# joshuacwnewton/swiftwatcher

Measured on AMD Instinct MI355X. Metric: frames/sec (segment+classify) on 1080p ROI batches, higher is better.
Workload: dtype f64 (image_filtering), f32 (CNN)

## Files before the change

swiftwatcher_amd/csrc/cnn_poolsq.hip:

```cpp
#include "cnn_common.h"

namespace swk {

template <int PT, int NB>
__global__ __launch_bounds__(64 * PT * NB) void k_pool_squeeze(const float *__restrict__ src, int n, int T, int C, int P, const float *__restrict__ wgt,
                                                               const float *__restrict__ bias, int S, float *__restrict__ dst, int dH, int dW, int dC,
                                                               int off_y, int off_x, const float *__restrict__ ring, int live_lo, int live_n)
{
    constexpr int NW = PT * NB, NT = 64 * NW, PP = 32 * PT + 1, SP = 32 * NB + 1, KC = 32;
    __shared__ float sB[2][KC * PP];
    __shared__ float sA[2][KC * SP];
    const int tid = threadIdx.x, lane = tid & 63, wave = tid >> 6, r = lane & 31, hh = lane >> 5;
    const int pt = wave % PT, nb = wave / PT;
    const int npix = P * P, nchunk = C / KC;
    const int64_t rs = (int64_t)T * C;

    auto stage = [&](int seg, int c, int buf) {
        const int kb = c * KC;
        for (int i = tid; i < 32 * NB * 8; i += NT) {
            const int co = i >> 3, q = i & 7;
            float4 w = make_float4(0.f, 0.f, 0.f, 0.f);
            if (co < S) w = *(const float4 *)(wgt + (int64_t)co * C + kb + 4 * q);
            float *a = &sA[buf][(4 * q) * SP + co];
            a[0] = w.x; a[SP] = w.y; a[2 * SP] = w.z; a[3 * SP] = w.w;
        }
        const float *base = src + (int64_t)seg * T * rs + kb, *rbase = ring + kb;
        for (int i = tid; i < 32 * PT * 8; i += NT) {
            const int p = i >> 3, q = i & 7;
            float4 m = make_float4(0.f, 0.f, 0.f, 0.f);
            if (p < npix) {
                const int py = p / P, px = p - py * P;
                const int64_t o0 = (int64_t)(2 * py) * rs + (int64_t)(2 * px) * C + 4 * q;
                bool iny[3], inx[3];
#pragma unroll
                for (int d = 0; d < 3; ++d) {
                    iny[d] = (unsigned)(2 * py + d - live_lo) < (unsigned)live_n;
                    inx[d] = (unsigned)(2 * px + d - live_lo) < (unsigned)live_n;
                }
                m = *(const float4 *)((iny[0] && inx[0] ? base : rbase) + o0);
#pragma unroll
                for (int dy = 0; dy < 3; ++dy)
#pragma unroll
                    for (int dx = 0; dx < 3; ++dx) {
                        if (dy == 0 && dx == 0) continue;
                        const float4 v = *(const float4 *)((iny[dy] && inx[dx] ? base : rbase) + o0 + dy * rs + dx * C);
                        m.x = fmaxf(m.x, v.x); m.y = fmaxf(m.y, v.y); m.z = fmaxf(m.z, v.z); m.w = fmaxf(m.w, v.w);
                    }
            }
            float *b = &sB[buf][(4 * q) * PP + p];
            b[0] = m.x; b[PP] = m.y; b[2 * PP] = m.z; b[3 * PP] = m.w;
        }
    };

    for (int seg = blockIdx.x; seg < n; seg += gridDim.x) {
        f16v acc;
#pragma unroll
        for (int e = 0; e < 16; ++e) acc[e] = 0.0f;
        stage(seg, 0, 0);
        __syncthreads();
        for (int c = 0; c < nchunk; ++c) {
            const int buf = c & 1;
            if (c + 1 < nchunk) stage(seg, c + 1, buf ^ 1);
            const float *a = &sA[buf][(16 * hh) * SP + 32 * nb + r];
            const float *b = &sB[buf][(16 * hh) * PP + 32 * pt + r];
#pragma unroll
            for (int i = 0; i < 16; ++i) acc = __builtin_amdgcn_mfma_f32_32x32x2f32(a[i * SP], b[i * PP], acc, 0, 0, 0);
            __syncthreads();
        }
        const int p = 32 * pt + r;
        if (p < npix) {
            const int py = p / P, px = p - py * P;
            float *o = dst + (((int64_t)seg * dH + off_y + py) * dW + off_x + px) * dC + 32 * nb + 4 * hh;
#pragma unroll
            for (int g = 0; g < 4; ++g) {
                const int co = 32 * nb + 8 * g + 4 * hh;
                if (co < S) store_bias_relu(o + 8 * g, acc, g, *(const float4 *)(bias + co));
            }
        }
    }
}

template <int PT, int NB>
static int launch_pool_squeeze(hipStream_t s, const float *src, int n, int T, int C, int P, const float *wgt, const float *bias, int S, const Place &pl,
                               const float *ring, int live_lo, int live_n)
{
    int blocks = n < 256 * 8 ? n : 256 * 8;
    hipLaunchKernelGGL((k_pool_squeeze<PT, NB>), dim3((unsigned)blocks), dim3(64 * PT * NB), 0, s, src, n, T, C, P, wgt, bias, S, pl.dst, pl.dH, pl.dW,
                       pl.dC, pl.off_y, pl.off_x, ring, live_lo, live_n);
    return hipGetLastError() == hipSuccess ? SWK_OK : SWK_ERR_HIP;
}

}

#pragma GCC visibility push(default)
extern "C" {

int32_t swk_nhwc_maxpool3s2_conv1x1_bias_relu_place(void *stream, const float *src, int32_t n, int32_t t, int32_t cin, const float *weight,
                                                    const float *bias, int32_t cout, float *dst, int32_t dH, int32_t dW, int32_t dC,
                                                    int32_t off_y, int32_t off_x, const float *ring, int32_t live_lo, int32_t live_n)
{
    const int P = (t - 3) / 2 + 1;
    const swk::Place pl{dst, dH, dW, dC, off_y, off_x, 0};
    if (!src || !weight || !bias || n < 1 || t < 3 || cin < 32 || (cin & 31) || cout > 64 || P * P > 96 || !swk::place_ok(pl, P, P, cout, true) ||
        (((uintptr_t)src | (uintptr_t)weight | (uintptr_t)bias) & 15))
        return SWK_ERR_ARG;
    if (!ring) { ring = src; live_lo = 0; live_n = t; }
    if (live_lo < 0 || live_n < 0 || live_lo + live_n > t || ((uintptr_t)ring & 15)) return SWK_ERR_ARG;
    using namespace swk;
    hipStream_t s = (hipStream_t)stream;
    const int PT = (P * P + 31) / 32, NB = (cout + 31) / 32;
    if (PT == 1 && NB == 1) return launch_pool_squeeze<1, 1>(s, src, n, t, cin, P, weight, bias, cout, pl, ring, live_lo, live_n);
    if (PT == 2 && NB == 1) return launch_pool_squeeze<2, 1>(s, src, n, t, cin, P, weight, bias, cout, pl, ring, live_lo, live_n);
    if (PT == 3 && NB == 1) return launch_pool_squeeze<3, 1>(s, src, n, t, cin, P, weight, bias, cout, pl, ring, live_lo, live_n);
    if (PT == 1 && NB == 2) return launch_pool_squeeze<1, 2>(s, src, n, t, cin, P, weight, bias, cout, pl, ring, live_lo, live_n);
    if (PT == 2 && NB == 2) return launch_pool_squeeze<2, 2>(s, src, n, t, cin, P, weight, bias, cout, pl, ring, live_lo, live_n);
    if (PT == 3 && NB == 2) return launch_pool_squeeze<3, 2>(s, src, n, t, cin, P, weight, bias, cout, pl, ring, live_lo, live_n);
    return SWK_ERR_ARG;
}

}
#pragma GCC visibility pop
```

Baseline: 42590.

## Add persistent row-tiled maxpool+squeeze kernel with LDS-resident weights and pipelined loads

Adds a new fused maxpool3s2 + 1x1 conv kernel. It flattens all pooled pixels across segments into 32-row tiles, one tile per wave. Weights and bias are loaded once into dynamic LDS per persistent block. The 3x3 window loads are software-pipelined against the MFMA steps using sched_group_barriers, and magic-number division is used for pixel indexing. The aim is to stop restaging weights for every segment, fix poor wave utilisation when P*P is not a multiple of 32, and hide global load latency. The new path runs only for large batches that fit in LDS; otherwise the old per-segment kernel is used. It adds heavy register and LDS pressure and complexity.

```diff
diff --git a/swiftwatcher_amd/csrc/cnn_poolsq.hip b/swiftwatcher_amd/csrc/cnn_poolsq.hip
--- a/swiftwatcher_amd/csrc/cnn_poolsq.hip
+++ b/swiftwatcher_amd/csrc/cnn_poolsq.hip
@@ -2,10 +2,186 @@
 
 namespace swk {
 
+constexpr int POOLSQ_XP = 34;
+constexpr int POOLSQ_XFLOATS = 32 * POOLSQ_XP;
+
+template <int NBLK, int NWV>
+__global__ __launch_bounds__(64 * NWV, 3) void k_pool_squeeze(const float *__restrict__ src, int64_t rows, int T, int C, const float *__restrict__ wgt,
+                                                              const float *__restrict__ bias, int S, float *__restrict__ dst, int dH, int dW, int dC,
+                                                              int off_y, int off_x, const float *__restrict__ ring, int live_lo, int live_n,
+                                                              FastDiv fpp, FastDiv fp)
+{
+    constexpr int NP = 32 * NBLK, PITCH = NP + 1, NT = 64 * NWV, KC = 32, XP = POOLSQ_XP;
+    extern __shared__ float lds[];
+    const int tid = threadIdx.x, lane = tid & 63, r = lane & 31, hh = lane >> 5, q = lane & 7, pl = lane >> 3;
+    const int wave = __builtin_amdgcn_readfirstlane(tid >> 6);
+    float *lbias = lds + ((C * PITCH + 3) & ~3);
+    float *xw = lbias + NP + wave * POOLSQ_XFLOATS + (4 * q) * XP + pl;
+    const float *xr = lbias + NP + wave * POOLSQ_XFLOATS + (16 * hh) * XP + r;
+    const int P = (int)fp.d, nchunk = C / KC;
+    const int rs = T * C;
+    const int64_t ntiles = (rows + 31) >> 5, stride = (int64_t)gridDim.x * NWV;
+    int64_t tile = (int64_t)blockIdx.x * NWV + wave;
+
+    const float *lsrc[4];
+    int lwin[4];
+    unsigned lmask[4];
+    int lk = 0;
+    auto pixel = [&](unsigned t32, int j, unsigned &seg, unsigned &py, unsigned &px) -> bool {
+        asm volatile("" : "+s"(t32));
+        const unsigned m = t32 * 32u + (unsigned)j;
+        const bool valid = m < (unsigned)rows;
+        const unsigned mm = valid ? m : (unsigned)rows - 1u;
+        seg = fpp.div(mm);
+        const unsigned p = mm - seg * fpp.d;
+        py = fp.div(p);
+        px = p - py * (unsigned)P;
+        return valid;
+    };
+    auto locate = [&](int64_t t) {
+        int l = threadIdx.x & 63;
+        asm volatile("" : "+v"(l));
+#pragma unroll
+        for (int u = 0; u < 4; ++u) {
+            unsigned seg, py, px;
+            pixel((unsigned)t, 8 * u + (l >> 3), seg, py, px);
+            lwin[u] = (int)(2 * py) * rs + (int)(2 * px) * C + 4 * (l & 7);
+            lsrc[u] = src + (int64_t)seg * T * rs + lwin[u];
+            unsigned iny = 0, inx = 0;
+#pragma unroll
+            for (int d = 0; d < 3; ++d) {
+                iny |= (unsigned)((unsigned)(2 * py + d - live_lo) < (unsigned)live_n) << d;
+                inx |= (unsigned)((unsigned)(2 * px + d - live_lo) < (unsigned)live_n) << d;
+            }
+            lmask[u] = ((iny & 1u) ? inx : 0u) | ((iny & 2u) ? inx << 3 : 0u) | ((iny & 4u) ? inx << 6 : 0u);
+        }
+    };
+    float4 L[3][4];
+    float4 m[4];
+    auto issue = [&](int dy) {
+#pragma unroll
+        for (int u = 0; u < 4; ++u)
+#pragma unroll
+            for (int dx = 0; dx < 3; ++dx)
+                L[dx][u] = *(const float4 *)((((lmask[u] >> (3 * dy + dx)) & 1u) ? lsrc[u] : ring + lwin[u]) + (lk + dy * rs + dx * C));
+    };
+    auto max4 = [](const float4 a, const float4 b) { return make_float4(fmaxf(a.x, b.x), fmaxf(a.y, b.y), fmaxf(a.z, b.z), fmaxf(a.w, b.w)); };
+    auto fold = [&](bool first) {
+#pragma unroll
+        for (int u = 0; u < 4; ++u) m[u] = max4(max4(first ? L[0][u] : max4(m[u], L[0][u]), L[1][u]), L[2][u]);
+    };
+
+    locate(tile < ntiles ? tile : ntiles - 1);
+    issue(0);
+    for (int co = tid >> 4; co < NP; co += NT / 16)
+        for (int c4 = (tid & 15) * 4; c4 < C; c4 += 64) {
+            const float4 wv = co < S ? *(const float4 *)(wgt + (int64_t)co * C + c4) : make_float4(0.0f, 0.0f, 0.0f, 0.0f);
+            float *w = lds + c4 * PITCH + co;
+            w[0] = wv.x; w[PITCH] = wv.y; w[2 * PITCH] = wv.z; w[3 * PITCH] = wv.w;
+        }
+    for (int i = tid; i < NP; i += NT) lbias[i] = i < S ? bias[i] : 0.0f;
+    fold(true);
+    issue(1);
+    fold(false);
+    issue(2);
+    __syncthreads();
+
+    const float *wrow0 = lds + (16 * hh) * PITCH + r, *wrow = wrow0;
+    float bw[2][NBLK], bx[2];
+
+#define SWK_PS_STEPS(I0, I1)                                                                                                          \
+    _Pragma("unroll") for (int i = I0; i < I1; ++i) {                                                                                 \
+        if (i < 15) {                                                                                                                 \
+            _Pragma("unroll") for (int nb = 0; nb < NBLK; ++nb) bw[(i + 1) & 1][nb] = wrow[(i + 1) * PITCH + 32 * nb];                \
+            bx[(i + 1) & 1] = xr[(i + 1) * XP];                                                                                       \
+        }                                                                                                                             \
+        _Pragma("unroll") for (int nb = 0; nb < NBLK; ++nb) acc[nb] = __builtin_amdgcn_mfma_f32_32x32x2f32(bw[i & 1][nb], bx[i & 1], acc[nb], 0, 0, 0); \
+        if (i < 15) __builtin_amdgcn_sched_group_barrier(0x100 , NBLK + 1, 0);                                           \
+        __builtin_amdgcn_sched_group_barrier(0x008 , NBLK, 0);                                                              \
+    }
+
+    for (; tile < ntiles; tile += stride) {
+        const bool more = tile + stride < ntiles;
+        f16v acc[NBLK];
+#pragma unroll
+        for (int nb = 0; nb < NBLK; ++nb)
+#pragma unroll
+            for (int e = 0; e < 16; ++e) acc[nb][e] = 0.0f;
+        for (int c = 0; c < nchunk; ++c) {
+            fold(false);
+#pragma unroll
+            for (int u = 0; u < 4; ++u) {
+                xw[8 * u] = m[u].x; xw[XP + 8 * u] = m[u].y; xw[2 * XP + 8 * u] = m[u].z; xw[3 * XP + 8 * u] = m[u].w;
+            }
+            __builtin_amdgcn_wave_barrier();
+#pragma unroll
+            for (int nb = 0; nb < NBLK; ++nb) bw[0][nb] = wrow[32 * nb];
+            bx[0] = xr[0];
+            const bool last = c + 1 == nchunk;
+            if (!last) lk += KC;
+            else { lk = 0; locate(more ? tile + stride : tile); }
+            __builtin_amdgcn_sched_barrier(0);
+            issue(0);
+            __builtin_amdgcn_sched_barrier(0);
+            SWK_PS_STEPS(0, 5)
+            __builtin_amdgcn_sched_barrier(0);
+            fold(true);
+            issue(1);
+            __builtin_amdgcn_sched_barrier(0);
+            SWK_PS_STEPS(5, 10)
+            __builtin_amdgcn_sched_barrier(0);
+            fold(false);
+            issue(2);
+            __builtin_amdgcn_sched_barrier(0);
+            SWK_PS_STEPS(10, 16)
+            __builtin_amdgcn_sched_barrier(0);
+            wrow = last ? wrow0 : wrow + KC * PITCH;
+        }
+        unsigned seg, py, px;
+        int h4 = lane;
+        asm volatile("" : "+v"(h4));
+        const int rr = h4 & 31;
+        h4 = (h4 >> 5) * 4;
+        if (pixel((unsigned)tile, rr, seg, py, px)) {
+            float *o = dst + (((int64_t)seg * dH + off_y + py) * dW + off_x + px) * (int64_t)dC + h4;
+#pragma unroll
+            for (int nb = 0; nb < NBLK; ++nb)
+#pragma unroll
+                for (int g = 0; g < 4; ++g) {
+                    const int co = nb * 32 + 8 * g;
+                    if (co + h4 < S) store_bias_relu(o + co, acc[nb], g, *(const float4 *)(lbias + co + h4));
+                }
+        }
+    }
+#undef SWK_PS_STEPS
+}
+
+static size_t pool_squeeze_lds(int C, int nblk, int nwv)
+{
+    return (size_t)(((C * (32 * nblk + 1) + 3) & ~3) + 32 * nblk + nwv * POOLSQ_XFLOATS) * sizeof(float);
+}
+
+template <int NBLK, int NWV>
+static int launch_pool_squeeze_w(hipStream_t s, const float *src, int64_t rows, int T, int C, int P, const float *wgt, const float *bias, int S,
+                                 const Place &pl, const float *ring, int live_lo, int live_n)
+{
+    const size_t lds = pool_squeeze_lds(C, NBLK, NWV);
+    static unsigned long long attr_mask = 0;
+    if (!ensure_dyn_lds((const void *)k_pool_squeeze<NBLK, NWV>, 160 * 1024 - 256, attr_mask)) return SWK_ERR_HIP;
+    const int64_t ntiles = (rows + 31) / 32;
+    int64_t blocks = (ntiles + NWV - 1) / NWV;
+    const int64_t by_lds = (int64_t)((160 * 1024 - 256) / lds), by_waves = 12 / NWV;
+    const int64_t cap = 256 * (by_lds < by_waves ? by_lds : by_waves);
+    if (blocks > cap) blocks = cap;
+    hipLaunchKernelGGL((k_pool_squeeze<NBLK, NWV>), dim3((unsigned)blocks), dim3(64 * NWV), lds, s, src, rows, T, C, wgt, bias, S, pl.dst, pl.dH, pl.dW,
+                       pl.dC, pl.off_y, pl.off_x, ring, live_lo, live_n, FastDiv((unsigned)(P * P)), FastDiv((unsigned)P));
+    return hipGetLastError() == hipSuccess ? SWK_OK : SWK_ERR_HIP;
+}
+
 template <int PT, int NB>
-__global__ __launch_bounds__(64 * PT * NB) void k_pool_squeeze(const float *__restrict__ src, int n, int T, int C, int P, const float *__restrict__ wgt,
-                                                               const float *__restrict__ bias, int S, float *__restrict__ dst, int dH, int dW, int dC,
-                                                               int off_y, int off_x, const float *__restrict__ ring, int live_lo, int live_n)
+__global__ __launch_bounds__(64 * PT * NB) void k_pool_squeeze_seg(const float *__restrict__ src, int n, int T, int C, int P, const float *__restrict__ wgt,
+                                                                   const float *__restrict__ bias, int S, float *__restrict__ dst, int dH, int dW, int dC,
+                                                                   int off_y, int off_x, const float *__restrict__ ring, int live_lo, int live_n)
 {
     constexpr int NW = PT * NB, NT = 64 * NW, PP = 32 * PT + 1, SP = 32 * NB + 1, KC = 32;
     __shared__ float sB[2][KC * PP];
@@ -81,13 +257,32 @@
 }
 
 template <int PT, int NB>
-static int launch_pool_squeeze(hipStream_t s, const float *src, int n, int T, int C, int P, const float *wgt, const float *bias, int S, const Place &pl,
-                               const float *ring, int live_lo, int live_n)
+static int launch_pool_squeeze_seg(hipStream_t s, const float *src, int n, int T, int C, int P, const float *wgt, const float *bias, int S, const Place &pl,
+                                   const float *ring, int live_lo, int live_n)
 {
     int blocks = n < 256 * 8 ? n : 256 * 8;
-    hipLaunchKernelGGL((k_pool_squeeze<PT, NB>), dim3((unsigned)blocks), dim3(64 * PT * NB), 0, s, src, n, T, C, P, wgt, bias, S, pl.dst, pl.dH, pl.dW,
+    hipLaunchKernelGGL((k_pool_squeeze_seg<PT, NB>), dim3((unsigned)blocks), dim3(64 * PT * NB), 0, s, src, n, T, C, P, wgt, bias, S, pl.dst, pl.dH, pl.dW,
                        pl.dC, pl.off_y, pl.off_x, ring, live_lo, live_n);
     return hipGetLastError() == hipSuccess ? SWK_OK : SWK_ERR_HIP;
+}
+
+
+static bool pool_squeeze_by_row_tiles(int n, int P, int C, int nblk, int &nwv)
+{
+    const int64_t rows = (int64_t)n * P * P, ntiles = (rows + 31) / 32;
+    nwv = 12;
+    while (nwv > 3 && pool_squeeze_lds(C, nblk, nwv) > 160 * 1024 - 256) nwv /= 2;
+    return pool_squeeze_lds(C, nblk, nwv) <= 160 * 1024 - 256 && rows <= (int64_t)0x7fffff00 && ntiles >= 2 * 256 * nwv;
+}
+
+template <int NBLK>
+static int launch_pool_squeeze(hipStream_t s, const float *src, int n, int T, int C, int P, int nwv, const float *wgt, const float *bias, int S,
+                               const Place &pl, const float *ring, int live_lo, int live_n)
+{
+    const int64_t rows = (int64_t)n * P * P;
+    if (nwv == 12) return launch_pool_squeeze_w<NBLK, 12>(s, src, rows, T, C, P, wgt, bias, S, pl, ring, live_lo, live_n);
+    if (nwv == 6) return launch_pool_squeeze_w<NBLK, 6>(s, src, rows, T, C, P, wgt, bias, S, pl, ring, live_lo, live_n);
+    return launch_pool_squeeze_w<NBLK, 3>(s, src, rows, T, C, P, wgt, bias, S, pl, ring, live_lo, live_n);
 }
 
 }
@@ -109,12 +304,17 @@
     using namespace swk;
     hipStream_t s = (hipStream_t)stream;
     const int PT = (P * P + 31) / 32, NB = (cout + 31) / 32;
-    if (PT == 1 && NB == 1) return launch_pool_squeeze<1, 1>(s, src, n, t, cin, P, weight, bias, cout, pl, ring, live_lo, live_n);
-    if (PT == 2 && NB == 1) return launch_pool_squeeze<2, 1>(s, src, n, t, cin, P, weight, bias, cout, pl, ring, live_lo, live_n);
-    if (PT == 3 && NB == 1) return launch_pool_squeeze<3, 1>(s, src, n, t, cin, P, weight, bias, cout, pl, ring, live_lo, live_n);
-    if (PT == 1 && NB == 2) return launch_pool_squeeze<1, 2>(s, src, n, t, cin, P, weight, bias, cout, pl, ring, live_lo, live_n);
-    if (PT == 2 && NB == 2) return launch_pool_squeeze<2, 2>(s, src, n, t, cin, P, weight, bias, cout, pl, ring, live_lo, live_n);
-    if (PT == 3 && NB == 2) return launch_pool_squeeze<3, 2>(s, src, n, t, cin, P, weight, bias, cout, pl, ring, live_lo, live_n);
+    int nwv;
+    if (pool_squeeze_by_row_tiles(n, P, cin, NB, nwv)) {
+        if (NB == 1) return launch_pool_squeeze<1>(s, src, n, t, cin, P, nwv, weight, bias, cout, pl, ring, live_lo, live_n);
+        return launch_pool_squeeze<2>(s, src, n, t, cin, P, nwv, weight, bias, cout, pl, ring, live_lo, live_n);
+    }
+    if (PT == 1 && NB == 1) return launch_pool_squeeze_seg<1, 1>(s, src, n, t, cin, P, weight, bias, cout, pl, ring, live_lo, live_n);
+    if (PT == 2 && NB == 1) return launch_pool_squeeze_seg<2, 1>(s, src, n, t, cin, P, weight, bias, cout, pl, ring, live_lo, live_n);
+    if (PT == 3 && NB == 1) return launch_pool_squeeze_seg<3, 1>(s, src, n, t, cin, P, weight, bias, cout, pl, ring, live_lo, live_n);
+    if (PT == 1 && NB == 2) return launch_pool_squeeze_seg<1, 2>(s, src, n, t, cin, P, weight, bias, cout, pl, ring, live_lo, live_n);
+    if (PT == 2 && NB == 2) return launch_pool_squeeze_seg<2, 2>(s, src, n, t, cin, P, weight, bias, cout, pl, ring, live_lo, live_n);
+    if (PT == 3 && NB == 2) return launch_pool_squeeze_seg<3, 2>(s, src, n, t, cin, P, weight, bias, cout, pl, ring, live_lo, live_n);
     return SWK_ERR_ARG;
 }
 
```

Measured after the change: 43070 (median of 6 runs). 1.01x the previous value.
